# deu439/ARFlow

Measured on AMD Instinct MI355X. Metric: image-pairs/sec fwd+bwd, PWCLite 384x640 bs=8, higher is better.
Workload: dtype f32; 1 GPU; pwclite_uflow+uflow_loss, 384x640 pairs, batch 8 per GPU, fwd(both directions)+loss+bwd+allreduce+Adam; global_batch=8, parallelism=dp1, step_start=seeded weights + fresh Adam state, restored before every step, loss_finite=True

## Files before the change

arflow_amd/_lib.py:

```python
import ctypes
import os

_HERE = os.path.dirname(os.path.abspath(__file__))
LIB_PATH = os.path.join(_HERE, 'csrc', 'libarflow_hip.so')

c_fp = ctypes.c_void_p
c_i = ctypes.c_int
c_l = ctypes.c_long
c_f = ctypes.c_float
c_d = ctypes.c_double

PROTOTYPES = {
    'arflow_abi_version': [],
    'arflow_take_stale_error': [],
    'arflow_set_deterministic': [c_i],
    'arflow_get_deterministic': [],
    'arflow_flow_up_fwd': [c_fp, c_fp, c_i, c_i, c_i, c_i, c_i, c_fp],
    'arflow_flow_up_bwd': [c_fp, c_fp, c_i, c_i, c_i, c_i, c_i, c_fp],
    'arflow_out_up2_fwd': [c_fp, c_l, c_fp, c_l, c_i, c_i, c_i, c_i, c_i, c_i, c_f, c_fp],
    'arflow_out_up2_bwd': [c_fp, c_l, c_fp, c_l, c_i, c_i, c_i, c_i, c_i, c_fp],
    'arflow_out_tail_fwd': [c_fp, c_l, c_fp, c_fp, c_i, c_i, c_i, c_i, c_i, c_i, c_f, c_fp],
    'arflow_prob_up_fwd': [c_fp, c_l, c_fp, c_l, c_i, c_i, c_i, c_i, c_i, c_i, c_i, c_f, c_fp],
    'arflow_prob_up_bwd': [c_fp, c_l, c_fp, c_l, c_i, c_i, c_i, c_i, c_i, c_i, c_fp],
    'arflow_profile_marker': [c_i, c_fp],
    'arflow_sums_rows': [c_i, c_i, c_i],
    'arflow_corr_fwd': [c_fp, c_fp, c_fp, c_fp, c_i, c_i, c_i, c_i, c_i, c_f, c_fp],
    'arflow_corr_sign_planes': [c_i, c_i, c_i],
    'arflow_corr_strided_supported': [c_i, c_i, c_i],
    'arflow_corr_fwd_strided': [c_fp, c_fp, c_fp, c_l, c_fp, c_i, c_i, c_i, c_i, c_i, c_f, c_fp],
    'arflow_corr_bwd_strided': [c_fp, c_l, c_fp, c_l, c_fp, c_fp, c_fp, c_fp, c_fp, c_i, c_i, c_i, c_i, c_i, c_f, c_fp],
    'arflow_corr_bwd': [c_fp, c_fp, c_fp, c_fp, c_fp, c_fp, c_fp, c_i, c_i, c_i, c_i, c_i, c_f, c_fp],
    'arflow_corr_fwd_bf16': [c_fp, c_fp, c_fp, c_i, c_i, c_i, c_i, c_i, c_f, c_fp],
    'arflow_corr_bwd_bf16': [c_fp, c_fp, c_fp, c_fp, c_fp, c_fp, c_i, c_i, c_i, c_i, c_i, c_f, c_fp],
    'arflow_warp_fwd_bf16': [c_fp, c_fp, c_fp, c_fp, c_i, c_i, c_i, c_i, c_i, c_i, c_l, c_i, c_i, c_i, c_fp],
    'arflow_warp_bwd_bf16': [c_fp, c_fp, c_fp, c_fp, c_fp, c_i, c_i, c_i, c_i, c_i, c_i, c_l, c_i, c_i, c_i, c_fp],
    'arflow_warp_nearest_fwd': [c_fp, c_fp, c_fp, c_i, c_i, c_i, c_i, c_i, c_i, c_l, c_i, c_i, c_i, c_fp],
    'arflow_warp_nearest_bwd': [c_fp, c_fp, c_fp, c_i, c_i, c_i, c_i, c_i, c_i, c_l, c_i, c_i, c_i, c_fp],
    'arflow_warp_bicubic_fwd': [c_fp, c_fp, c_fp, c_i, c_i, c_i, c_i, c_i, c_i, c_l, c_i, c_i, c_i, c_fp],
    'arflow_warp_bicubic_bwd': [c_fp, c_fp, c_fp, c_fp, c_fp, c_i, c_i, c_i, c_i, c_i, c_i, c_l, c_i, c_i, c_i, c_fp],
    'arflow_ssim_fwd': [c_fp, c_fp, c_fp, c_i, c_i, c_i, c_i, c_i, c_fp],
    'arflow_ssim_bwd': [c_fp, c_fp, c_fp, c_fp, c_i, c_i, c_i, c_i, c_i, c_fp],
    'arflow_corr_general_out_size': [c_i, c_i, c_i, c_i, c_i, c_i, c_i, c_fp, c_fp, c_fp],
    'arflow_corr_general_fwd': [c_fp, c_fp, c_fp, c_i, c_i, c_i, c_i, c_i, c_i, c_i, c_i, c_i, c_fp],
    'arflow_corr_general_bwd': [c_fp, c_fp, c_fp, c_fp, c_fp, c_i, c_i, c_i, c_i, c_i, c_i, c_i, c_i, c_i, c_fp],
    'arflow_featnorm_fwd': [c_fp, c_fp, c_fp, c_fp, c_fp, c_fp, c_i, c_l, c_i, c_fp],
    'arflow_featnorm_bwd': [c_fp, c_fp, c_fp, c_fp, c_fp, c_fp, c_fp, c_fp, c_i, c_l, c_i, c_fp],
    'arflow_level_supported': [c_i, c_i, c_i],
    'arflow_level_bwd_ws_bytes': [c_i, c_i, c_i, c_i],
    'arflow_level_fwd': [c_fp, c_fp, c_fp, c_l, c_i, c_i, c_fp, c_fp, c_l, c_fp, c_i, c_fp, c_l, c_fp, c_l, c_fp, c_fp, c_fp, c_i, c_i, c_i, c_i, c_i, c_f, c_i, c_i, c_i, c_fp],
    'arflow_level_bwd': [c_fp, c_l, c_fp, c_fp, c_l, c_fp, c_l, c_fp, c_fp, c_fp, c_fp, c_l, c_fp, c_l, c_fp, c_fp, c_i, c_fp, c_fp, c_fp, c_i, c_i, c_fp, c_i, c_i, c_i, c_i, c_i, c_f, c_i, c_i, c_i, c_fp],
    'arflow_level_fwd_m': [c_fp, c_fp, c_fp, c_l, c_i, c_i, c_fp, c_fp, c_l, c_fp, c_i, c_fp, c_l, c_fp, c_l, c_fp, c_fp, c_fp, c_fp, c_i, c_fp, c_i, c_i, c_i, c_i, c_i, c_i, c_f, c_i, c_i, c_i, c_fp],
    'arflow_up2_bwd': [c_fp, c_fp, c_i, c_i, c_i, c_i, c_fp],
    'arflow_bias_act_mom_rows': [c_i, c_l],
    'arflow_bias_act_fwd_mom': [c_fp, c_fp, c_fp, c_fp, c_i, c_i, c_l, c_f, c_fp],
    'arflow_level_acc_rows': [c_i, c_i, c_i, c_i, c_i],
    'arflow_level_moments': [c_fp, c_fp, c_fp, c_i, c_l, c_fp],
    'arflow_level_warp_fwd': [c_fp, c_fp, c_fp, c_l, c_i, c_i, c_fp, c_fp, c_l, c_fp, c_fp, c_i, c_i, c_i, c_i, c_i, c_i, c_i, c_fp],
    'arflow_level_corr_fwd': [c_fp, c_fp, c_fp, c_i, c_i, c_fp, c_l, c_fp, c_l, c_fp, c_fp, c_i, c_i, c_i, c_i, c_i, c_f, c_fp],
    'arflow_level_corr_bwd': [c_fp, c_l, c_fp, c_fp, c_l, c_fp, c_fp, c_fp, c_fp, c_i, c_i, c_i, c_i, c_i, c_f, c_fp],
    'arflow_bias_act_fwd': [c_fp, c_fp, c_fp, c_i, c_i, c_l, c_f, c_fp],
    'arflow_bias_act_bwd': [c_fp, c_fp, c_fp, c_fp, c_i, c_i, c_l, c_f, c_fp],
    'arflow_headconv_fwd': [c_fp, c_fp, c_fp, c_fp, c_i, c_i, c_i, c_i, c_fp],
    'arflow_headconv_bwd_data': [c_fp, c_fp, c_fp, c_i, c_i, c_i, c_i, c_fp],
    'arflow_headconv_bwd_weight_ws_bytes': [c_i, c_i, c_i, c_i],
    'arflow_headconv_bwd_weight': [c_fp, c_fp, c_fp, c_fp, c_fp, c_i, c_i, c_i, c_i, c_fp],
    'arflow_splitconv_pack_bytes': [c_i, c_i],
    'arflow_splitconv_pack': [c_fp, c_fp, c_i, c_i, c_i, c_fp],
    'arflow_splitconv_fwd': [c_fp, c_fp, c_fp, c_i, c_i, c_i, c_i, c_i, c_fp],
    'arflow_splitconv_fwd_ex': [c_fp, c_l, c_fp, c_fp, c_l, c_fp, c_i, c_f, c_i, c_i, c_i, c_i, c_i, c_fp],
    'arflow_splitconv_wgrad_ws_bytes': [c_i, c_i, c_i, c_i, c_i],
    'arflow_splitconv_wgrad': [c_fp, c_l, c_fp, c_l, c_fp, c_fp, c_i, c_i, c_i, c_i, c_i, c_fp],
    'arflow_dense_cat_fwd': [c_fp, c_fp, c_fp, c_fp, c_i, c_i, c_i, c_l, c_f, c_fp],
    'arflow_dense_gbias_rows': [c_i, c_l],
    'arflow_dense_grad_gather': [c_fp, c_i, c_fp, c_l, c_fp, c_fp, c_i, c_i, c_l, c_f, c_fp],
    'arflow_warp_fwd': [c_fp, c_fp, c_fp, c_fp, c_i, c_i, c_i, c_i, c_i, c_i, c_l, c_i, c_i, c_i, c_fp],
    'arflow_warp_bwd': [c_fp, c_fp, c_fp, c_fp, c_fp, c_i, c_i, c_i, c_i, c_i, c_i, c_l, c_i, c_i, c_i, c_fp],
    'arflow_splat_map': [c_fp, c_fp, c_i, c_i, c_i, c_l, c_i, c_fp],
    'arflow_coord_mask': [c_fp, c_fp, c_i, c_i, c_i, c_l, c_i, c_fp],
    'arflow_occ_bidir': [c_fp, c_fp, c_fp, c_i, c_i, c_i, c_l, c_l, c_f, c_f, c_fp],
    'arflow_census_fwd': [c_fp, c_fp, c_fp, c_fp, c_fp, c_fp, c_i, c_i, c_i, c_i, c_fp],
    'arflow_census_bwd': [c_fp, c_fp, c_fp, c_fp, c_fp, c_i, c_i, c_i, c_i, c_fp],
    'arflow_census_warp_supported': [c_i, c_i],
    'arflow_census_warp_fwd': [c_fp, c_fp, c_fp, c_l, c_fp, c_fp, c_fp, c_fp, c_i, c_i, c_i, c_i, c_fp],
    'arflow_census_warp_bwd': [c_fp, c_fp, c_fp, c_l, c_fp, c_fp, c_fp, c_i, c_i, c_i, c_i, c_fp],
    'arflow_census_warp_pair_fwd': [c_fp, c_fp, c_l, c_fp, c_fp, c_fp, c_fp, c_i, c_i, c_i, c_i, c_fp],
    'arflow_census_warp_pair_bwd': [c_fp, c_fp, c_l, c_fp, c_fp, c_fp, c_i, c_i, c_i, c_i, c_fp],
    'arflow_uflow_pair_bwd': [c_fp, c_fp, c_l, c_fp, c_fp, c_fp, c_i, c_i, c_i, c_i, c_fp, c_l, c_fp, c_fp, c_fp, c_i, c_i, c_f, c_f, c_i, c_i, c_i, c_fp],
    'arflow_down4_gray_z': [c_fp, c_fp, c_fp, c_fp, c_i, c_i, c_i, c_fp],
    'arflow_splat_smooth_fwd': [c_fp, c_fp, c_fp, c_fp, c_i, c_i, c_i, c_l, c_f, c_f, c_i, c_i, c_i, c_i, c_fp],
    'arflow_down4_gray': [c_fp, c_fp, c_fp, c_i, c_i, c_i, c_fp],
    'arflow_photo_fwd': [c_fp, c_fp, c_fp, c_fp, c_fp, c_i, c_i, c_i, c_i, c_fp],
    'arflow_photo_bwd': [c_fp, c_fp, c_fp, c_fp, c_fp, c_fp, c_i, c_i, c_i, c_i, c_fp],
    'arflow_photo_warp_rows': [c_i, c_i, c_i],
    'arflow_photo_warp_fwd': [c_fp, c_l, c_l, c_fp, c_l, c_l, c_fp, c_l, c_l, c_fp, c_l, c_l, c_i, c_i, c_i, c_i, c_fp, c_fp, c_i, c_i, c_i, c_i, c_i, c_i, c_fp],
    'arflow_photo_warp_bwd': [c_fp, c_l, c_l, c_fp, c_l, c_l, c_fp, c_l, c_l, c_fp, c_l, c_l, c_i, c_i, c_i, c_i, c_fp, c_fp, c_l, c_l, c_i, c_i, c_i, c_i, c_i, c_i, c_fp],
    'arflow_area_pyramid_ws_bytes': [c_i, c_i, c_i, c_fp, c_i],
    'arflow_area_pyramid': [c_fp, c_fp, c_i, c_i, c_i, c_fp, c_i, c_fp],
    'arflow_smooth_fwd': [c_fp, c_fp, c_fp, c_i, c_i, c_i, c_i, c_l, c_f, c_f, c_i, c_i, c_i, c_fp],
    'arflow_smooth_bwd': [c_fp, c_fp, c_fp, c_fp, c_i, c_i, c_i, c_i, c_l, c_f, c_f, c_i, c_i, c_i, c_fp],
    'arflow_down4': [c_fp, c_fp, c_i, c_i, c_i, c_fp],
    'arflow_up4_clamp_mul': [c_fp, c_fp, c_fp, c_i, c_i, c_i, c_fp],
    'arflow_flow_eval_rows': [c_i, c_i],
    'arflow_flow_eval': [c_fp, c_fp, c_fp, c_fp, c_fp, c_i, c_i, c_i, c_i, c_i, c_i, c_fp],
    'arflow_triag_solve': [c_fp, c_fp, c_fp, c_fp, c_fp, c_fp, c_i, c_i, c_i, c_i, c_fp],
    'arflow_triag_solve_bwd': [c_fp, c_fp, c_fp, c_fp, c_fp, c_fp, c_fp, c_fp, c_fp, c_fp, c_fp, c_i, c_i, c_i, c_i, c_fp],
    'arflow_triag_inverse_diagonal': [c_fp, c_fp, c_fp, c_fp, c_i, c_i, c_i, c_fp],
    'arflow_band_mv_fwd': [c_fp, c_l, c_fp, c_l, c_fp, c_l, c_fp, c_l, c_fp, c_l, c_i, c_i, c_i, c_i, c_i, c_i, c_fp],
    'arflow_band_mv_bwd': [c_fp, c_l, c_fp, c_l, c_fp, c_l, c_fp, c_l, c_fp, c_l, c_fp, c_l, c_fp, c_l, c_fp, c_l, c_i, c_i, c_i, c_i, c_i, c_i, c_fp],
    'arflow_lowrank_sample_fwd': [c_fp, c_l, c_fp, c_l, c_fp, c_fp, c_l, c_i, c_i, c_i, c_i, c_i, c_fp],
    'arflow_lowrank_work_size': [c_i, c_i, c_i, c_i],
    'arflow_lowrank_logdet_fwd': [c_fp, c_l, c_fp, c_fp, c_fp, c_i, c_i, c_i, c_i, c_fp],
    'arflow_lowrank_bwd': [c_fp, c_l, c_fp, c_fp, c_l, c_fp, c_fp, c_fp, c_l, c_fp, c_l, c_i, c_i, c_i, c_i, c_i, c_fp],
    'arflow_mixture_work_size': [c_i, c_i, c_i, c_i, c_i],
    'arflow_mixture_sample_fwd': [c_fp, c_l, c_fp, c_l, c_fp, c_l, c_fp, c_fp, c_l, c_fp, c_i, c_i, c_i, c_i, c_i, c_fp],
    'arflow_mixture_logpdf_fwd': [c_fp, c_fp, c_fp, c_fp, c_fp, c_i, c_i, c_i, c_i, c_i, c_fp],
    'arflow_mixture_bwd': [c_fp, c_l, c_fp, c_l, c_fp, c_l, c_fp, c_fp, c_fp, c_fp, c_l, c_fp, c_l, c_fp, c_l, c_i, c_i, c_i, c_i, c_i, c_fp],
    'arflow_mixture_entropy_map': [c_fp, c_l, c_fp, c_l, c_fp, c_fp, c_fp, c_l, c_fp, c_i, c_i, c_i, c_i, c_i, c_fp],
    'arflow_gauss_pyr_work_size': [c_fp, c_fp, c_i, c_i],
    'arflow_gauss_pyr_sample_fwd': [c_fp, c_fp, c_fp, c_fp, c_fp, c_fp, c_fp, c_fp, c_i, c_i, c_fp, c_fp, c_fp],
    'arflow_gauss_pyr_sample_bwd': [c_fp, c_fp, c_fp, c_fp, c_fp, c_fp, c_fp, c_fp, c_fp, c_fp, c_fp, c_i, c_i, c_fp],
    'arflow_mse_work_size': [c_i, c_i, c_i],
    'arflow_mse_fwd': [c_fp, c_l, c_i, c_fp, c_l, c_i, c_i, c_fp, c_l, c_i, c_i, c_i, c_i, c_i, c_i, c_fp, c_fp, c_fp],
    'arflow_mse_bwd': [c_fp, c_l, c_i, c_fp, c_l, c_i, c_i, c_fp, c_l, c_fp, c_fp, c_l, c_fp, c_l, c_i, c_i, c_i, c_i, c_i, c_i, c_fp],
    'arflow_resize_flow': [c_fp, c_l, c_i, c_i, c_fp, c_l, c_i, c_i, c_i, c_i, c_fp],
# ... 56 lines not shown
```

arflow_amd/csrc/split_tiles.hpp:

```cpp
#pragma once
#include <array>

namespace splitbf16 {
inline int tiles32(int n) { return (n + 31) / 32; }
constexpr int MAX_KT = 2;

struct TilePart { int kt, count, first; };
inline std::array<TilePart, 2> split_tiles(int n, int max_t) {
  const int chunks = (n + max_t - 1) / max_t, base = n / chunks, extra = n % chunks;
  return {{{base + 1, extra, 0}, {base, chunks - extra, extra * (base + 1)}}};
}
}
```

arflow_amd/csrc/splitconv.hip:

```cpp
#include <climits>
#include <cstdint>

#include "splitbf16.hpp"

namespace {
using namespace splitbf16;

constexpr int NT = 256;
constexpr int CB = 32;
constexpr int PLANE_BYTES = CB * 2;
constexpr int PIX_BYTES = 3 * PLANE_BYTES + 16;
constexpr int FRAG = 64 * 8;

template <int PW>
struct Geo {
  static constexpr int PR = 32 / PW;
  static constexpr int TH = 8 * PR;
  static constexpr int HW = PW + 2;
  static constexpr int HH = TH + 2;
  static constexpr int NPIX = HH * HW;
  static constexpr int LDS_BYTES = NPIX * PIX_BYTES;
};

__global__ __launch_bounds__(NT) void splitconv_pack_kernel(const float* __restrict__ w, bf16x8* __restrict__ packed, int wK, int wC,
// ... 237 lines not shown
int launch(const Ends& ends, const bf16x8* packed, int N, int C, int K, int H, int W, int kt_first, int chunks, hipStream_t st) {
  using G = Geo<PW>;
  if (const int rc = allow_dynamic_lds<&splitconv_kernel<KT, PW>>(G::LDS_BYTES)) return rc;
  const int tx = (W + PW - 1) / PW, ty = (H + G::TH - 1) / G::TH;
  const dim3 grid((unsigned)((long)N * tx * ty), (unsigned)chunks);
  hipLaunchKernelGGL((splitconv_kernel<KT, PW>), grid, dim3(NT), G::LDS_BYTES, st, ends.x, ends.x_bs, packed, ends.y, ends.y_bs, ends.bias,
                     ends.act, ends.slope, C, K, H, W, tiles32(K), 2 * tiles32(C), kt_first, tx, ty);
  return af_launch_status();
}

template <int PW>
int launch_kt(int KT, const Ends& e, const bf16x8* packed, int N, int C, int K, int H, int W, int kt_first, int chunks,
              hipStream_t st) {
  return KT == 1 ? launch<1, PW>(e, packed, N, C, K, H, W, kt_first, chunks, st)
                 : launch<2, PW>(e, packed, N, C, K, H, W, kt_first, chunks, st);
}
}

extern "C" long arflow_splitconv_pack_bytes(int K, int C) {
  if (!pack_shape_ok(K, C)) return ARFLOW_ESHAPE;
  return (long)3 * 9 * tiles32(K) * 2 * tiles32(C) * FRAG * 2;
}

extern "C" int arflow_splitconv_pack(const float* w, void* packed, int K, int C, int transpose_flip, arflow_stream_t stream) {
  af_clear_stale_error();
  AF_REQUIRE_PTR(w);
  AF_REQUIRE_PTR(packed);
  AF_REQUIRE(pack_shape_ok(K, C), ARFLOW_ESHAPE);
  AF_REQUIRE(transpose_flip == 0 || transpose_flip == 1, ARFLOW_EPARAM);
  AF_REQUIRE(((uintptr_t)packed & 15) == 0, ARFLOW_EPARAM);
  const int Kout = transpose_flip ? C : K, Cin = transpose_flip ? K : C;
  const int nkt = tiles32(Kout), ncs = 2 * tiles32(Cin);
  const int nfrag = 9 * nkt * ncs * 64;
  hipLaunchKernelGGL(splitconv_pack_kernel, dim3((unsigned)af_cdiv(nfrag, NT)), dim3(NT), 0, (hipStream_t)stream, w,
                     (bf16x8*)packed, K, C, Kout, Cin, nkt, ncs, transpose_flip);
  return af_launch_status();
}

extern "C" int arflow_splitconv_fwd_ex(const float* x, long x_bstride, const void* packed, float* y, long y_bstride,
                                       const float* bias, int act, float negative_slope, int N, int C, int K, int H, int W,
                                       arflow_stream_t stream) {
  af_clear_stale_error();
  AF_REQUIRE_PTR(x);
  AF_REQUIRE_PTR(packed);
  AF_REQUIRE_PTR(y);
  AF_REQUIRE(N > 0 && C > 0 && K > 0 && H > 0 && W > 0, ARFLOW_ESHAPE);
  AF_REQUIRE((long)N * C * H * W <= INT_MAX && (long)N * K * H * W <= INT_MAX && pack_shape_ok(K, C), ARFLOW_ESHAPE);
  AF_REQUIRE(x_bstride >= (long)C * H * W && y_bstride >= (long)K * H * W, ARFLOW_ESHAPE);
  AF_REQUIRE(x_bstride <= INT_MAX / N && y_bstride <= INT_MAX / N, ARFLOW_ESHAPE);
  AF_REQUIRE(act == 0 || act == 1, ARFLOW_EPARAM);
  AF_REQUIRE(act == 1 || bias == nullptr, ARFLOW_EPARAM);
  AF_REQUIRE(((uintptr_t)packed & 15) == 0, ARFLOW_EPARAM);
  const Ends ends{x, x_bstride, y, y_bstride, bias, act, negative_slope};
  const auto waste = [&](int pw) {
    const int th = 8 * (32 / pw);
    return (long)((W + pw - 1) / pw * pw) * ((H + th - 1) / th * th);
  };
  int PW = 32;
  if (waste(16) < waste(PW)) PW = 16;
  if (waste(8) < waste(PW)) PW = 8;
  const bf16x8* pk = (const bf16x8*)packed;
  hipStream_t st = (hipStream_t)stream;
  for (const TilePart& p : split_tiles(tiles32(K), MAX_KT)) {
    if (p.count == 0) continue;
    int rc;
    if (PW == 32) rc = launch_kt<32>(p.kt, ends, pk, N, C, K, H, W, p.first, p.count, st);
    else if (PW == 16) rc = launch_kt<16>(p.kt, ends, pk, N, C, K, H, W, p.first, p.count, st);
    else rc = launch_kt<8>(p.kt, ends, pk, N, C, K, H, W, p.first, p.count, st);
    if (rc != ARFLOW_OK) return rc;
  }
  return ARFLOW_OK;
}

extern "C" int arflow_splitconv_fwd(const float* x, const void* packed, float* y, int N, int C, int K, int H, int W,
                                    arflow_stream_t stream) {
  return arflow_splitconv_fwd_ex(x, (long)C * H * W, packed, y, (long)K * H * W, nullptr, 0, 0.f, N, C, K, H, W, stream);
}
```

arflow_amd/functional.py:

```python
import contextlib

import torch

from . import _lib
from . import ddp as _ddp

PAD = {'zeros': 0, 'border': 1}
NORM_ARFLOW, NORM_UFLOW = 0, 1


def _need_gpu(*tensors):
    for t in tensors:
        if t is None:
            continue
        if not t.is_cuda:
            raise _lib.ArflowHipError('arflow_amd ops run on the GPU only (got a %s tensor); there is no CPU '
                                      'fallback -- the CPU oracle lives in oracle/ and is test-only' % t.device)
        if t.dtype != torch.float32:
            raise _lib.ArflowHipError('arflow_amd ops are fp32 only (got %s)' % t.dtype)


def _p(t):
    return None if t is None else t.data_ptr()

# ... 874 lines not shown
            ctx.save_for_backward(*xs, *ws, w_head)
        ctx.slope, ctx.inplace = slope, inplace
        ctx.set_materialize_grads(False)
        return x6, flow

    @staticmethod
    @torch.autograd.function.once_differentiable
    def backward(ctx, gx6, gflow):
        if ctx.inplace:
            x6, ws, w_head = ctx.saved_tensors[0], ctx.saved_tensors[1:6], ctx.saved_tensors[6]
            tail = [int(w.shape[0]) for w in ws]
            xs = [x6[:, sum(tail[m:]):] for m in range(5)] + [x6]
        else:
            xs, ws, w_head = ctx.saved_tensors[:6], ctx.saved_tensors[6:11], ctx.saved_tensors[11]
        need = ctx.needs_input_grad
        grads = [None] * 14
        if gx6 is None and gflow is None:
            return tuple(grads)
        x6 = xs[5]
        B, C6, H, W = x6.shape
        ocs = [int(w.shape[0]) for w in ws]
        lowest = 0 if need[0] else next((m for m in range(1, 6) if need[2 * m] or need[2 * m + 1]), 6)
        dx_head = None
        if gflow is not None:
            gflow = gflow.contiguous()
            if lowest < 6:
                dx_head = _headconv_dgrad(gflow, w_head, x6)
            grads[12], grads[13] = _headconv_wgrad(x6, gflow, w_head, need[12], need[13])
        if lowest == 6:
            return tuple(grads)
        top = [t for t in (gx6, dx_head) if t is not None]
        dxs = []
        for m in range(5, max(lowest, 1) - 1, -1):
            srcs = [(t, sum(ocs[m:5]), None) for t in top] + [(dx, sum(ocs[m:k - 1]), None) for dx, k in dxs]
            gy, gb = dense_grad_gather(srcs, ocs[m - 1], act=xs[m], slope=ctx.slope, want_bias=need[2 * m + 1])
            want_dx, want_dw = m > lowest, bool(need[2 * m])
            xm = xs[m - 1]
            dx_native = want_dx and splitconv_takes(B, ocs[m - 1], xm.shape[1], H, W)
            dw_native = want_dw and (_inplace_wgrad_takes if ctx.inplace else splitconv_wgrad_takes)(B, xm.shape[1], ocs[m - 1], H, W)
            dx, dw = _conv3x3_grads(xm, ws[m - 1], gy, want_dx, want_dw, dx_native, dw_native)
            grads[2 * m], grads[2 * m + 1] = dw, gb
            if want_dx:
                dxs.append((dx, m))
        if need[0]:
            srcs = [(t, sum(ocs), None) for t in top] + [(dx, sum(ocs[:k - 1]), None) for dx, k in dxs]
            grads[0] = dense_grad_gather(srcs, int(xs[0].shape[1]))[0]
        return tuple(grads)


def dense_estimator(x, slope, params):
    return DenseEstimatorFunction.apply(x, slope, *params)


@_samples_mode
class BiasLeakyReLUMomentsFunction(torch.autograd.Function):

    @staticmethod
    def forward(ctx, x, bias, slope):
        _need_gpu(x)
        if not x.is_contiguous():
            raise ValueError('bias_leaky_relu expects a contiguous [B,C,...] tensor')
        B, C = x.shape[0], x.shape[1]
        hw = x[0, 0].numel()
        if bias is not None:
            _need_gpu(bias)
            bias = bias.contiguous()
        rows = _lib.load().arflow_bias_act_mom_rows(C, hw)
        mom = torch.empty(B, rows, 2, device=x.device, dtype=torch.float64)
        with torch.cuda.device_of(x):
            _call('arflow_bias_act_fwd_mom', _p(x), _p(bias), _p(x), _p(mom), B, C, hw, float(slope), _stream(), key=(B, C, hw))
        ctx.mark_dirty(x)
        ctx.mark_non_differentiable(mom)
        ctx.save_for_backward(x)
        ctx.slope, ctx.has_bias = float(slope), bias is not None
        return x, mom

    @staticmethod
    def backward(ctx, gout, gmom_unused):
        y, = ctx.saved_tensors
        B, C = y.shape[0], y.shape[1]
        hw = y[0, 0].numel()
        gout = gout.contiguous()
        gin = torch.empty_like(gout)
        gb = torch.empty(C, device=y.device, dtype=torch.float32) if (ctx.has_bias and ctx.needs_input_grad[1]) else None
        with torch.cuda.device_of(y):
            _call('arflow_bias_act_bwd', _p(gout), _p(y), _p(gin), _p(gb), B, C, hw, ctx.slope, _stream(), key=(B, C, hw))
        return gin, gb, None


def bias_leaky_relu_moments(x, bias, slope=0.1):
    return BiasLeakyReLUMomentsFunction.apply(x, bias, slope)


@_samples_mode
class WarpFunction(torch.autograd.Function):

    @staticmethod
    def forward(ctx, src, flow, pad, align_corners, norm, want_valid=False):
        _need_gpu(src, flow)
        src = src.contiguous()
        flow, fbs = _flow_view(flow)
        B, C, Hs, Ws = src.shape
        _, _, H, W = flow.shape
        if flow.shape[0] != B:
            raise ValueError('batch mismatch between source and flow')
        out = torch.empty(B, C, H, W, device=src.device, dtype=torch.float32)
# ... 1041 lines not shown
```

arflow_amd/models/blocks.py:

```python
import torch
import torch.nn as nn
import torch.nn.functional as F

from .. import functional as AF

bias_act = AF.bias_leaky_relu


class ConvAct(nn.Sequential):

    want_moments = False
    last_moments = None

    def split_route(self, x):
        if not self._split_kind(x):
            return False, False
        c = self[0]
        N, C, H, W = x.shape
        return AF.splitconv_takes(N, C, c.out_channels, H, W), AF.splitconv_takes(N, c.out_channels, C, H, W)

    def split_wgrad_route(self, x):
        if not self._split_kind(x):
            return False
        N, C, H, W = x.shape
# ... 78 lines not shown

    def __init__(self, ch_in, ch_out=2):
        super().__init__()
        self.conv1 = conv(ch_in, 128)
        self.conv2 = conv(ch_in + 128, 128)
        self.conv3 = conv(ch_in + 256, 96)
        self.conv4 = conv(ch_in + 352, 64)
        self.conv5 = conv(ch_in + 416, 32)
        self.feat_dim = ch_in + 448
        self.conv_last = conv(ch_in + 448, ch_out, isReLU=False)

    def native(self, x):
        return AF.dense_block_enabled() and self.conv_last.native(x) and self.conv1[0].weight.dtype == torch.float32

    def forward(self, x):
        layers = (self.conv1, self.conv2, self.conv3, self.conv4, self.conv5)
        if self.native(x):
            params = [p for layer in layers + (self.conv_last,) for p in (layer[0].weight, layer[0].bias)]
            return AF.dense_estimator(x, self.conv1[1].negative_slope, params)
        for layer in layers:
            x = torch.cat([layer(x), x], dim=1)
        return x, self.conv_last(x)


class FlowEstimatorReduce(nn.Module):

    def __init__(self, ch_in, ch_out=2):
        super().__init__()
        self.conv1 = conv(ch_in, 128)
        self.conv2 = conv(128, 128)
        self.conv3 = conv(128 + 128, 96)
        self.conv4 = conv(128 + 96, 64)
        self.conv5 = conv(96 + 64, 32)
        self.feat_dim = 32
        self.predict_flow = conv(64 + 32, ch_out, isReLU=False)

    def forward(self, x):
        x1 = self.conv1(x)
        x2 = self.conv2(x1)
        x3 = self.conv3(torch.cat([x1, x2], dim=1))
        x4 = self.conv4(torch.cat([x2, x3], dim=1))
        x5 = self.conv5(torch.cat([x3, x4], dim=1))
        return x5, self.predict_flow(torch.cat([x4, x5], dim=1))


class ContextNetwork(nn.Module):

    def __init__(self, ch_in, ch_out=2):
        super().__init__()
        self.convs = nn.Sequential(
            conv(ch_in, 128, 3, 1, 1), conv(128, 128, 3, 1, 2), conv(128, 128, 3, 1, 4), conv(128, 96, 3, 1, 8),
            conv(96, 64, 3, 1, 16), conv(64, 32, 3, 1, 1), conv(32, ch_out, isReLU=False))

    def forward(self, x):
        return self.convs(x)


def init_conv_weights(module, scheme):
    for layer in module.modules():
        if isinstance(layer, (nn.Conv2d, nn.ConvTranspose2d)):
            if scheme == 'kaiming':
                nn.init.kaiming_normal_(layer.weight)
            else:
                nn.init.xavier_uniform_(layer.weight)
            if layer.bias is not None:
                nn.init.constant_(layer.bias, 0)


def level_drops(training, rate, n, n_passes, batch_per_pass, device):
    if not (training and rate > 0):
        return None
    vals = [[float(torch.rand(1) > rate) for _ in range(n)] for _ in range(n_passes)]
    t = torch.tensor(vals, dtype=torch.float32)
    t = t.repeat_interleave(batch_per_pass, dim=0).t().contiguous()
    return t.to(device, non_blocking=True).view(n, -1, 1, 1, 1)


def pair_pass(pyr_all, moms, B, with_bk, run):
    have_m = moms is not None and all(t is not None for t in moms)
    if with_bk:
        swapped = [torch.cat([p[B:], p[:B]], 0) for p in pyr_all]
        m = (list(moms), [torch.roll(t, B, 0) for t in moms]) if have_m else None
        flows = run(list(pyr_all), swapped, 2, m)
        return {'flows_fw': [f[:B] for f in flows], 'flows_bw': [f[B:] for f in flows]}
    m = ([t[:B] for t in moms], [t[B:] for t in moms]) if have_m else None
    return {'flows_fw': run([p[:B] for p in pyr_all], [p[B:] for p in pyr_all], 1, m)}
```

include/arflow_hip.h:

```cpp
#ifndef ARFLOW_HIP_H
#define ARFLOW_HIP_H

#ifdef __cplusplus
extern "C" {
#endif

typedef void* arflow_stream_t;

#define ARFLOW_OK 0
#define ARFLOW_ENULL (-1001)
#define ARFLOW_ESHAPE (-1002)
#define ARFLOW_EPARAM (-1003)
#define ARFLOW_ENONDET (-1004)
#define ARFLOW_ELAUNCH_BASE (-2000)

#define ARFLOW_PAD_ZEROS 0
#define ARFLOW_PAD_BORDER 1

#define ARFLOW_NORM_ARFLOW 0
#define ARFLOW_NORM_UFLOW 1
#define ARFLOW_NORM_UFLOW_ABS 2
#define ARFLOW_COORDS_ABS 2

#define ARFLOW_SUM_COLS 4
// ... 56 lines not shown
int arflow_level_fwd_m(const float* x1, const float* x2, const float* flow, long flow_bstride, int flow_is_coarse,
                       int up_align_corners, float* flow_up, float* flow_up2, long flow_up2_bstride, float* x2w, int norm_mode,
                       float* out, long out_bstride, float* x1n, long x1n_bstride, unsigned* sign_bits, float* stats,
                       double* acc, const double* x1_rows, int x1_nrows, const double* x2_rows, int x2_nrows, int B, int C, int H,
                       int W, int max_disp, float negative_slope, int pad_mode, int align_corners, int coord_norm,
                       arflow_stream_t stream);
int arflow_level_bwd(const float* gout, long gout_bstride, const unsigned* sign_bits, const float* x1n, long x1n_bstride,
                     const float* gx1n_direct, long gx1n_direct_bstride, const float* x1, const float* x2, const float* x2w,
                     const float* flow_full, long flow_bstride, const float* gflow_a, long gflow_a_bstride,
                     const float* gflow_b, const float* stats, int norm_mode, float* gx1, float* gx2, float* gflow,
                     int flow_is_coarse, int up_align_corners, void* workspace, int B, int C, int H, int W, int max_disp,
                     float negative_slope, int pad_mode, int align_corners, int coord_norm, arflow_stream_t stream);
int arflow_level_acc_rows(int B, int C, int H, int W, int has_flow);
int arflow_up2_bwd(const float* gfine, float* gcoarse, int B, int H, int W, int up_align_corners, arflow_stream_t stream);
int arflow_level_moments(const float* x1, const float* x2, double* acc, int B, long n, arflow_stream_t stream);
int arflow_level_warp_fwd(const float* x1, const float* x2, const float* flow, long flow_bstride, int flow_is_coarse,
                          int up_align_corners, float* flow_up, float* flow_up2, long flow_up2_bstride, float* x2w,
                          double* acc, int B, int C, int H, int W, int pad_mode, int align_corners, int norm_mode,
                          arflow_stream_t stream);
int arflow_level_corr_fwd(const float* x1, const float* x2w, const double* acc, int acc_rows, int norm_mode, float* out,
                          long out_bstride, float* x1n, long x1n_bstride, unsigned* sign_bits, float* stats, int B, int C,
                          int H, int W, int max_disp, float negative_slope, arflow_stream_t stream);
int arflow_level_corr_bwd(const float* gout, long gout_bstride, const unsigned* sign_bits, const float* x1n,
                          long x1n_bstride, const float* x2w, const float* stats, float* gx1n, float* gx2n, int B, int C,
                          int H, int W, int max_disp, float negative_slope, arflow_stream_t stream);

int arflow_bias_act_fwd(const float* x, const float* bias, float* y, int B, int C, long HW,
                        float negative_slope, arflow_stream_t stream);
int arflow_bias_act_mom_rows(int C, long HW);
int arflow_bias_act_fwd_mom(const float* x, const float* bias, float* y, double* mom, int B, int C, long HW,
                            float negative_slope, arflow_stream_t stream);
int arflow_bias_act_bwd(const float* gout, const float* y, float* gin, float* gbias, int B, int C, long HW,
                        float negative_slope, arflow_stream_t stream);

int arflow_headconv_fwd(const float* x, const float* w, const float* bias, float* y, int B, int C, int H, int W,
                        arflow_stream_t stream);
int arflow_headconv_bwd_data(const float* dy, const float* w, float* dx, int B, int C, int H, int W,
                             arflow_stream_t stream);
long arflow_headconv_bwd_weight_ws_bytes(int B, int C, int H, int W);
int arflow_headconv_bwd_weight(const float* x, const float* dy, float* dw, float* dbias, void* ws, int B, int C, int H,
                               int W, arflow_stream_t stream);

long arflow_splitconv_pack_bytes(int K, int C);
int arflow_splitconv_pack(const float* w, void* packed, int K, int C, int transpose_flip, arflow_stream_t stream);
int arflow_splitconv_fwd(const float* x, const void* packed, float* y, int N, int C, int K, int H, int W,
                         arflow_stream_t stream);

int arflow_splitconv_fwd_ex(const float* x, long x_bstride, const void* packed, float* y, long y_bstride, const float* bias,
                            int act, float negative_slope, int N, int C, int K, int H, int W, arflow_stream_t stream);

long arflow_splitconv_wgrad_ws_bytes(int N, int C, int K, int H, int W);
int arflow_splitconv_wgrad(const float* x, long x_bstride, const float* dy, long dy_bstride, float* dw, void* ws, int N, int C,
                           int K, int H, int W, arflow_stream_t stream);

#define ARFLOW_DENSE_MAX_SRC 8
typedef struct {
  const float* ptr;
  long bstride;
  const float* scale;
} arflow_dense_src;
int arflow_dense_cat_fwd(const float* y, const float* bias, const float* x, float* out, int B, int oc, int C, long HW,
                         float negative_slope, arflow_stream_t stream);
int arflow_dense_gbias_rows(int B, long HW);
int arflow_dense_grad_gather(const arflow_dense_src* srcs, int n_src, const float* act, long act_bs, float* gy,
                             float* gbias_rows, int B, int oc, long HW, float negative_slope, arflow_stream_t stream);

int arflow_warp_fwd(const float* src, const float* flow, float* out, float* valid, int B, int C,
                    int Hs, int Ws, int H, int W, long flow_bstride, int pad_mode, int align_corners,
                    int norm_mode, arflow_stream_t stream);

int arflow_warp_bwd(const float* gout, const float* src, const float* flow, float* gsrc, float* gflow,
                    int B, int C, int Hs, int Ws, int H, int W, long flow_bstride, int pad_mode,
                    int align_corners, int norm_mode, arflow_stream_t stream);

int arflow_splat_map(const float* flow, float* out, int B, int H, int W, long flow_bstride,
                     int variant, arflow_stream_t stream);

int arflow_coord_mask(const float* flow, float* out, int B, int H, int W, long flow_bstride, int mode,
                      arflow_stream_t stream);

int arflow_occ_bidir(const float* flow12, const float* flow21, float* out, int B, int H, int W,
                     long bstride12, long bstride21, float scale, float bias, arflow_stream_t stream);

int arflow_census_fwd(const float* im_a, const float* im_b, const float* mask, float* ham, float* dham,
                      float* sums, int B, int H, int W, int radius, arflow_stream_t stream);

int arflow_census_bwd(const float* im_a, const float* im_b, const float* gham, const float* scale,
                      float* g_im_b, int B, int H, int W, int radius, arflow_stream_t stream);

int arflow_census_warp_supported(int H, int W);
int arflow_census_warp_fwd(const float* gray_a, const float* gray_b, const float* flow, long flow_bstride,
                           const float* occ_small, float* mask_out, float* dham, float* sums, int B, int H, int W,
                           int radius, arflow_stream_t stream);
int arflow_census_warp_bwd(const float* gray_a, const float* gray_b, const float* flow, long flow_bstride,
                           const float* dham, const float* scale, float* gflow, int B, int H, int W, int radius,
                           arflow_stream_t stream);
int arflow_census_warp_pair_fwd(const float* gray, const float* flow, long flow_bstride, const float* occ_small,
                                float* mask_out, float* dham, float* sums, int B2, int H, int W, int radius,
                                arflow_stream_t stream);
int arflow_census_warp_pair_bwd(const float* gray, const float* flow, long flow_bstride, const float* dham,
                                const float* scale2, float* gflow, int B2, int H, int W, int radius, arflow_stream_t stream);
int arflow_uflow_pair_bwd(const float* gray, const float* flow, long flow_bstride, const float* dham, const float* scale2,
                          float* gflow, int B2, int H, int W, int radius, const float* flow2, long flow2_bstride,
                          const float* img2, const float* coef2, float* gflow2, int h2, int w2, float flow_scale, float alpha,
                          int order, int wmode, int penalty, arflow_stream_t stream);
int arflow_down4_gray(const float* im, float* small, float* gray, int B, int H, int W, arflow_stream_t stream);
// ... 190 lines not shown
```

Before: 190.6 image-pairs/s.

## Run dilated context-network convs as dense convs in a phase-decomposed layout

Adds phase kernels that rearrange activations into a space-to-batch (phase-decomposed) layout, so each dilated 3x3 conv in the context network becomes an ordinary dense 3x3 conv. These can then run on the existing bf16-split splitconv kernel instead of the framework's dilated convolution path. A custom autograd function chains the four dilated layers. It fuses the phase reshuffle with the leaky-ReLU backward and the bias-gradient reduction, and falls back to MIOpen weight-gradient on the plain layout for some layers. The trade is extra layout-conversion passes, padding in the virtual layout, and more saved tensors, in exchange for faster dense conv kernels.

```diff
diff --git a/arflow_amd/_lib.py b/arflow_amd/_lib.py
--- a/arflow_amd/_lib.py
+++ b/arflow_amd/_lib.py
@@ -70,6 +70,10 @@
     'arflow_splitconv_fwd_ex': [c_fp, c_l, c_fp, c_fp, c_l, c_fp, c_i, c_f, c_i, c_i, c_i, c_i, c_i, c_fp],
     'arflow_splitconv_wgrad_ws_bytes': [c_i, c_i, c_i, c_i, c_i],
     'arflow_splitconv_wgrad': [c_fp, c_l, c_fp, c_l, c_fp, c_fp, c_i, c_i, c_i, c_i, c_i, c_fp],
+    'arflow_phase_layout': [c_i, c_i, c_i, c_i, c_fp],
+    'arflow_phase_rows': [c_i, c_i, c_i, c_i, c_i],
+    'arflow_phase_move': [c_fp, c_fp, c_fp, c_i, c_i, c_i, c_i, c_i, c_i, c_i, c_fp],
+    'arflow_phase_act_bwd': [c_fp, c_fp, c_fp, c_fp, c_fp, c_i, c_i, c_i, c_i, c_i, c_i, c_i, c_f, c_fp],
     'arflow_dense_cat_fwd': [c_fp, c_fp, c_fp, c_fp, c_i, c_i, c_i, c_l, c_f, c_fp],
     'arflow_dense_gbias_rows': [c_i, c_l],
     'arflow_dense_grad_gather': [c_fp, c_i, c_fp, c_l, c_fp, c_fp, c_i, c_i, c_l, c_f, c_fp],
diff --git a/arflow_amd/csrc/phase.hip b/arflow_amd/csrc/phase.hip
--- /dev/null
+++ b/arflow_amd/csrc/phase.hip
@@ -0,0 +1,174 @@
+#include <climits>
+
+#include "common.hpp"
+#include "phase_plan.hpp"
+
+namespace {
+using phase_plan::Plan;
+
+constexpr int NT = 256, NW = NT / 64;
+constexpr int RW = 8;
+constexpr int RB = RW * NW;
+constexpr int MAX_LDS = 160 * 1024 - 128;
+
+struct Ent {
+  int off;
+  int w;
+};
+struct Seg {
+  long base;
+  bool exists;
+};
+__device__ __forceinline__ Seg segments(const Plan& p, int C, int n, int c, int h) {
+  const phase_plan::Row r = phase_plan::row_to_virtual(p, h);
+  const long plane = (long)p.Hv * p.Wv;
+  Seg s;
+  s.exists = r.hv < p.Hv;
+  s.base = ((long)phase_plan::sample_to_virtual(p, n, r.g, 0) * C + c) * plane + (long)r.hv * p.Wv;
+  return s;
+}
+PHASE_HD inline int row_elements(const Plan& p) { return (p.d / p.Qg) * p.Wv; }
+PHASE_HD inline int named_rows(const Plan& p) { return (p.Pg == 1 ? p.Hs : p.Hs + 1) * p.d; }
+
+PHASE_HD inline int lds_column(int w) { return w + (w >> 5); }
+PHASE_HD inline int lds_pitch(int W) { return lds_column(W - 1) + 1; }
+
+__device__ __forceinline__ void column_map(const Plan& p, int C, Ent* __restrict__ tab) {
+  const int n = row_elements(p), step = C * p.Hv * p.Wv;
+  for (int t = threadIdx.x; t < n; t += NT) {
+    const int g = t / p.Wv, wv = t - g * p.Wv;
+    const int w = phase_plan::col_to_real(p, g, wv);
+    tab[t] = {g * step + wv, w < 0 ? -1 : lds_column(w)};
+  }
+}
+
+template <bool ACT>
+__global__ __launch_bounds__(NT) void phase_kernel(const float* __restrict__ src, const float* __restrict__ act, float* __restrict__ dst,
+                                                   float* __restrict__ dst2, double* __restrict__ rows, Plan ps, Plan pd, Plan pd2,
+                                                   int C, float slope) {
+  extern __shared__ __align__(8) float lds[];
+  __shared__ double red[NW];
+  const int lane = threadIdx.x & 63, wave = threadIdx.x >> 6;
+  const int c = blockIdx.y, n = blockIdx.z;
+  const int h0 = blockIdx.x * RB + wave * RW;
+  const int H = ps.H, W = lds_pitch(ps.W);
+  float* const mine = lds + (size_t)wave * RW * W;
+  const int nsrc = row_elements(ps), nd = row_elements(pd);
+  Ent* const tsrc = reinterpret_cast<Ent*>(lds + (size_t)RB * W);
+  Ent* const tdst = tsrc + nsrc;
+  Ent* const tdst2 = tdst + nd;
+  column_map(ps, C, tsrc);
+  column_map(pd, C, tdst);
+  if (dst2) column_map(pd2, C, tdst2);
+  __syncthreads();
+
+  double s[1] = {0.0};
+  if (h0 < H) {
+    long base[RW];
+#pragma unroll
+    for (int r = 0; r < RW; ++r) base[r] = segments(ps, C, n, c, min(h0 + r, H - 1)).base;
+    for (int t = lane; t < nsrc; t += 64) {
+      const Ent e = tsrc[t];
+      if (e.w < 0) continue;
+      float v[RW], a[RW];
+#pragma unroll
+      for (int r = 0; r < RW; ++r) {
+        v[r] = src[base[r] + e.off];
+        a[r] = ACT ? act[base[r] + e.off] : 1.f;
+      }
+#pragma unroll
+      for (int r = 0; r < RW; ++r) {
+        if (ACT) {
+          v[r] = a[r] > 0.f ? v[r] : v[r] * slope;
+          if (h0 + r < H) s[0] += (double)v[r];
+        }
+        mine[r * W + e.w] = v[r];
+      }
+    }
+  }
+  __syncthreads();
+
+  const auto put = [&](float* __restrict__ out, const Plan& p, const Ent* __restrict__ tab, int ne) {
+    const int hend = named_rows(p);
+    if (h0 >= hend) return;
+    Seg o[RW];
+#pragma unroll
+    for (int r = 0; r < RW; ++r) o[r] = segments(p, C, n, c, min(h0 + r, hend - 1));
+    for (int t = lane; t < ne; t += 64) {
+      const Ent e = tab[t];
+#pragma unroll
+      for (int r = 0; r < RW; ++r) {
+        if (h0 + r >= hend || !o[r].exists) continue;
+        out[o[r].base + e.off] = e.w >= 0 && h0 + r < H ? mine[r * W + e.w] : 0.f;
+      }
+    }
+  };
+  put(dst, pd, tdst, nd);
+  if (dst2) put(dst2, pd2, tdst2, row_elements(pd2));
+
+  if (ACT && rows) {
+    af_block_sum_f64<1, NT>(s, red);
+    if (threadIdx.x == 0) rows[((long)n * gridDim.x + blockIdx.x) * C + c] = s[0];
+  }
+}
+
+inline int walked_rows(const Plan& pd, const Plan* pd2) {
+  int h = named_rows(pd);
+  if (pd2 && named_rows(*pd2) > h) h = named_rows(*pd2);
+  return h;
+}
+inline bool layout_ok(int N, int C, int H, int W, int d) {
+  if (!(C > 0 && C <= 65535 && N <= 65535 && phase_plan::shape_ok(N, H, W, d))) return false;
+  return phase_plan::elements(phase_plan::make_plan(N, H, W, d), C) <= INT_MAX;
+}
+
+template <bool ACT>
+int launch(const float* src, const float* act, float* dst, float* dst2, double* rows, int N, int C, int H, int W, int d_src, int d_dst,
+           int d_dst2, float slope, hipStream_t st) {
+  AF_REQUIRE(layout_ok(N, C, H, W, d_src) && layout_ok(N, C, H, W, d_dst) && (!dst2 || layout_ok(N, C, H, W, d_dst2)), ARFLOW_ESHAPE);
+  const Plan ps = phase_plan::make_plan(N, H, W, d_src), pd = phase_plan::make_plan(N, H, W, d_dst);
+  const Plan pd2 = dst2 ? phase_plan::make_plan(N, H, W, d_dst2) : pd;
+  const long bytes = sizeof(float) * (long)RB * lds_pitch(W) + sizeof(Ent) * ((long)row_elements(ps) + row_elements(pd) + (dst2 ? row_elements(pd2) : 0));
+  AF_REQUIRE(bytes <= MAX_LDS, ARFLOW_ESHAPE);
+  if (bytes > 64 * 1024) {
+    const hipError_t e = hipFuncSetAttribute(reinterpret_cast<const void*>(&phase_kernel<ACT>), hipFuncAttributeMaxDynamicSharedMemorySize, MAX_LDS);
+    if (e != hipSuccess) return af_hip_status(e);
+  }
+  const dim3 grid((unsigned)af_cdiv(walked_rows(pd, dst2 ? &pd2 : nullptr), RB), (unsigned)C, (unsigned)N);
+  hipLaunchKernelGGL(phase_kernel<ACT>, grid, dim3(NT), (size_t)bytes, st, src, act, dst, dst2, rows, ps, pd, pd2, C, slope);
+  return af_launch_status();
+}
+}
+
+extern "C" int arflow_phase_layout(int N, int H, int W, int d, int* nv_hv_wv_pg_qg) {
+  AF_REQUIRE_PTR(nv_hv_wv_pg_qg);
+  AF_REQUIRE(phase_plan::shape_ok(N, H, W, d), ARFLOW_ESHAPE);
+  const Plan p = phase_plan::make_plan(N, H, W, d);
+  nv_hv_wv_pg_qg[0] = p.Nv, nv_hv_wv_pg_qg[1] = p.Hv, nv_hv_wv_pg_qg[2] = p.Wv, nv_hv_wv_pg_qg[3] = p.Pg, nv_hv_wv_pg_qg[4] = p.Qg;
+  return ARFLOW_OK;
+}
+
+extern "C" int arflow_phase_rows(int N, int H, int W, int d_dst, int d_dst2) {
+  AF_REQUIRE(phase_plan::shape_ok(N, H, W, d_dst) && (d_dst2 == 0 || phase_plan::shape_ok(N, H, W, d_dst2)), ARFLOW_ESHAPE);
+  const Plan pd = phase_plan::make_plan(N, H, W, d_dst), pd2 = phase_plan::make_plan(N, H, W, d_dst2 ? d_dst2 : d_dst);
+  return N * af_cdiv(walked_rows(pd, &pd2), RB);
+}
+
+extern "C" int arflow_phase_move(const float* src, float* dst, float* dst2, int N, int C, int H, int W, int d_src, int d_dst,
+                                 int d_dst2, arflow_stream_t stream) {
+  af_clear_stale_error();
+  AF_REQUIRE_PTR(src);
+  AF_REQUIRE_PTR(dst);
+  AF_REQUIRE((dst2 == nullptr) == (d_dst2 == 0), ARFLOW_EPARAM);
+  return launch<false>(src, nullptr, dst, dst2, nullptr, N, C, H, W, d_src, d_dst, d_dst2, 0.f, (hipStream_t)stream);
+}
+
+extern "C" int arflow_phase_act_bwd(const float* gout, const float* y, float* gin, float* gin2, double* rows, int N, int C, int H,
+                                    int W, int d_a, int d_b, int d_b2, float negative_slope, arflow_stream_t stream) {
+  af_clear_stale_error();
+  AF_REQUIRE_PTR(gout);
+  AF_REQUIRE_PTR(y);
+  AF_REQUIRE_PTR(gin);
+  AF_REQUIRE((gin2 == nullptr) == (d_b2 == 0), ARFLOW_EPARAM);
+  return launch<true>(gout, y, gin, gin2, rows, N, C, H, W, d_a, d_b, d_b2, negative_slope, (hipStream_t)stream);
+}
diff --git a/arflow_amd/csrc/phase_plan.hpp b/arflow_amd/csrc/phase_plan.hpp
--- /dev/null
+++ b/arflow_amd/csrc/phase_plan.hpp
@@ -0,0 +1,89 @@
+#pragma once
+#include <climits>
+
+#include "split_tiles.hpp"
+
+#if defined(__HIPCC__)
+#define PHASE_HD __host__ __device__
+#else
+#define PHASE_HD
+#endif
+
+namespace phase_plan {
+struct Plan {
+  int N, H, W, d;
+  int Pg, Qg;
+  int Hs, Ws;
+  int Hv, Wv, Nv;
+};
+
+inline bool shape_ok(int N, int H, int W, int d) { return N > 0 && H > 0 && W > 0 && d > 0 && d <= H && d <= W && (long)N * d * d <= INT_MAX; }
+
+inline Plan with_groups(int N, int H, int W, int d, int Pg, int Qg) {
+  Plan p;
+  p.N = N, p.H = H, p.W = W, p.d = d, p.Pg = Pg, p.Qg = Qg;
+  p.Hs = (H + d - 1) / d, p.Ws = (W + d - 1) / d;
+  p.Hv = Pg * (p.Hs + 1) - 1, p.Wv = Qg * (p.Ws + 1) - 1;
+  p.Nv = N * (d / Pg) * (d / Qg);
+  return p;
+}
+inline long tiled_pixels(const Plan& p) {
+  return (long)(p.d / p.Pg) * (p.d / p.Qg) * splitbf16::tile_pixels(p.Hv, p.Wv, splitbf16::pixel_tile_width(p.Hv, p.Wv));
+}
+inline Plan make_plan(int N, int H, int W, int d) {
+  Plan best = with_groups(N, H, W, d, 1, 1);
+  for (int Pg = 1; Pg <= d; ++Pg) {
+    if (d % Pg) continue;
+    for (int Qg = 1; Qg <= d; ++Qg) {
+      if (d % Qg) continue;
+      const Plan c = with_groups(N, H, W, d, Pg, Qg);
+      const long cc = tiled_pixels(c), cb = tiled_pixels(best);
+      if (cc < cb || (cc == cb && Pg * Qg < best.Pg * best.Qg)) best = c;
+    }
+  }
+  return best;
+}
+inline long elements(const Plan& p, int C) { return (long)p.Nv * C * p.Hv * p.Wv; }
+
+struct Row {
+  int g, hv;
+};
+PHASE_HD inline Row row_to_virtual(const Plan& p, int h) {
+  const int ph = h % p.d;
+  return {ph / p.Pg, (ph % p.Pg) * (p.Hs + 1) + h / p.d};
+}
+struct Col {
+  int g, wv;
+};
+PHASE_HD inline Col col_to_virtual(const Plan& p, int w) {
+  const int ph = w % p.d;
+  return {ph / p.Qg, (ph % p.Qg) * (p.Ws + 1) + w / p.d};
+}
+PHASE_HD inline int row_to_real(const Plan& p, int g, int hv) {
+  const int a = hv / (p.Hs + 1), i = hv % (p.Hs + 1);
+  const int h = i * p.d + g * p.Pg + a;
+  return i < p.Hs && h < p.H ? h : -1;
+}
+PHASE_HD inline int col_to_real(const Plan& p, int g, int wv) {
+  const int b = wv / (p.Ws + 1), j = wv % (p.Ws + 1);
+  const int w = j * p.d + g * p.Qg + b;
+  return j < p.Ws && w < p.W ? w : -1;
+}
+PHASE_HD inline int sample_to_virtual(const Plan& p, int n, int gp, int gq) { return (n * (p.d / p.Pg) + gp) * (p.d / p.Qg) + gq; }
+
+struct Pos {
+  int n, h, w;
+};
+PHASE_HD inline Pos to_virtual(const Plan& p, int n, int h, int w) {
+  const Row r = row_to_virtual(p, h);
+  const Col c = col_to_virtual(p, w);
+  return {sample_to_virtual(p, n, r.g, c.g), r.hv, c.wv};
+}
+PHASE_HD inline bool to_real(const Plan& p, int nv, int hv, int wv, Pos& o) {
+  const int nq = p.d / p.Qg, np = p.d / p.Pg;
+  const int h = row_to_real(p, (nv / nq) % np, hv), w = col_to_real(p, nv % nq, wv);
+  if (h < 0 || w < 0) return false;
+  o = {nv / (nq * np), h, w};
+  return true;
+}
+}
diff --git a/arflow_amd/csrc/split_tiles.hpp b/arflow_amd/csrc/split_tiles.hpp
--- a/arflow_amd/csrc/split_tiles.hpp
+++ b/arflow_amd/csrc/split_tiles.hpp
@@ -10,4 +10,15 @@
   const int chunks = (n + max_t - 1) / max_t, base = n / chunks, extra = n % chunks;
   return {{{base + 1, extra, 0}, {base, chunks - extra, extra * (base + 1)}}};
 }
+
+inline long tile_pixels(int H, int W, int pw) {
+  const int th = 8 * (32 / pw);
+  return (long)((W + pw - 1) / pw * pw) * ((H + th - 1) / th * th);
 }
+inline int pixel_tile_width(int H, int W) {
+  int pw = 32;
+  if (tile_pixels(H, W, 16) < tile_pixels(H, W, pw)) pw = 16;
+  if (tile_pixels(H, W, 8) < tile_pixels(H, W, pw)) pw = 8;
+  return pw;
+}
+}
diff --git a/arflow_amd/csrc/splitconv.hip b/arflow_amd/csrc/splitconv.hip
--- a/arflow_amd/csrc/splitconv.hip
+++ b/arflow_amd/csrc/splitconv.hip
@@ -313,13 +313,7 @@
   AF_REQUIRE(act == 1 || bias == nullptr, ARFLOW_EPARAM);
   AF_REQUIRE(((uintptr_t)packed & 15) == 0, ARFLOW_EPARAM);
   const Ends ends{x, x_bstride, y, y_bstride, bias, act, negative_slope};
-  const auto waste = [&](int pw) {
-    const int th = 8 * (32 / pw);
-    return (long)((W + pw - 1) / pw * pw) * ((H + th - 1) / th * th);
-  };
-  int PW = 32;
-  if (waste(16) < waste(PW)) PW = 16;
-  if (waste(8) < waste(PW)) PW = 8;
+  const int PW = pixel_tile_width(H, W);
   const bf16x8* pk = (const bf16x8*)packed;
   hipStream_t st = (hipStream_t)stream;
   for (const TilePart& p : split_tiles(tiles32(K), MAX_KT)) {
diff --git a/arflow_amd/functional.py b/arflow_amd/functional.py
--- a/arflow_amd/functional.py
+++ b/arflow_amd/functional.py
@@ -950,6 +950,146 @@
     return DenseEstimatorFunction.apply(x, slope, *params)
 
 
+_DILATED_CHAIN = __import__('os').environ.get('ARFLOW_DILATED_CHAIN', '1') != '0'
+DILATED_CHAIN_LAYERS = ((128, 128, 2), (128, 128, 4), (128, 96, 8), (96, 64, 16))
+_DILATED_WGRAD_NATIVE = (True, False, False, False)
+
+
+def dilated_chain_enabled():
+    return _DILATED_CHAIN
+
+
+def _dilated_wgrad_native():
+    env = __import__('os').environ.get('ARFLOW_DILATED_WGRAD')
+    if env and len(env) == 4 and set(env) <= {'0', '1'}:
+        return tuple(c == '1' for c in env)
+    return _DILATED_WGRAD_NATIVE
+
+
+def phase_layout(N, H, W, d):
+    import ctypes
+    out = (ctypes.c_int * 5)()
+    _lib.check(_lib.load().arflow_phase_layout(int(N), int(H), int(W), int(d), ctypes.cast(out, ctypes.c_void_p)), 'arflow_phase_layout')
+    return tuple(out)
+
+
+def _phase_empty(N, C, H, W, d, device):
+    if d == 1:
+        return torch.empty(N, C, H, W, device=device, dtype=torch.float32)
+    Nv, Hv, Wv, _, _ = phase_layout(N, H, W, d)
+    return torch.empty(Nv, C, Hv, Wv, device=device, dtype=torch.float32)
+
+
+def _phase_check(t, N, H, W, d, what):
+    _need_gpu(t)
+    Nv, Hv, Wv, _, _ = phase_layout(N, H, W, d)
+    if t.dim() != 4 or (t.shape[0], t.shape[2], t.shape[3]) != (Nv, Hv, Wv) or not t.is_contiguous():
+        raise ValueError('%s must be a contiguous [%d,C,%d,%d] tensor: layout %d of [%d,C,%d,%d]' % (what, Nv, Hv, Wv, d, N, H, W))
+
+
+def phase_move(src, real, d_src, d_dst, d_dst2=0, out=None, out2=None):
+    N, H, W = (int(v) for v in real)
+    _phase_check(src, N, H, W, d_src, 'phase_move: src')
+    C = int(src.shape[1])
+    dst = _phase_empty(N, C, H, W, d_dst, src.device) if out is None else out
+    dst2 = (_phase_empty(N, C, H, W, d_dst2, src.device) if out2 is None else out2) if d_dst2 else None
+    for t, d in ((out, d_dst), (out2 if d_dst2 else None, d_dst2)):
+        if t is not None:
+            _phase_check(t, N, H, W, d, 'phase_move: out')
+            if t.shape[1] != C:
+                raise ValueError('phase_move: out has %d channels, src %d' % (t.shape[1], C))
+    with torch.cuda.device_of(src):
+        _call('arflow_phase_move', _p(src), _p(dst), _p(dst2), N, C, H, W, int(d_src), int(d_dst), int(d_dst2), _stream())
+    return dst, dst2
+
+
+def phase_act_bwd(gout, y, real, d_a, d_b, d_b2=0, slope=0.1, want_bias=True):
+    N, H, W = (int(v) for v in real)
+    _phase_check(gout, N, H, W, d_a, 'phase_act_bwd: gout')
+    _phase_check(y, N, H, W, d_a, 'phase_act_bwd: y')
+    if y.shape != gout.shape:
+        raise ValueError('phase_act_bwd: gout and y differ in shape')
+    C = int(gout.shape[1])
+    gin = _phase_empty(N, C, H, W, d_b, gout.device)
+    gin2 = _phase_empty(N, C, H, W, d_b2, gout.device) if d_b2 else None
+    rows = None
+    if want_bias:
+        n = _lib.load().arflow_phase_rows(N, H, W, int(d_b), int(d_b2))
+        if n <= 0:
+            _lib.check(n, 'arflow_phase_rows')
+        rows = torch.empty(n, C, device=gout.device, dtype=torch.float64)
+    with torch.cuda.device_of(gout):
+        _call('arflow_phase_act_bwd', _p(gout), _p(y), _p(gin), _p(gin2), _p(rows), N, C, H, W, int(d_a), int(d_b), int(d_b2),
+              float(slope), _stream())
+    return gin, gin2, (None if rows is None else rows.sum(0).float())
+
+
+def _dilated_wgrad_miopen(x, gy, w, d):
+    args = [1, 1], [d, d], [d, d], False, [0, 0], 1
+    return torch.ops.aten.convolution_backward(gy, x, w, None, *args, [False, True, False])[1]
+
+
+class DilatedChainFunction(torch.autograd.Function):
+
+    @staticmethod
+    def forward(ctx, x, slope, *params):
+        if len(params) != 8:
+            raise ValueError('dilated_chain expects (w, b) of four layers')
+        _need_gpu(x, *params)
+        ws, bs = params[0::2], params[1::2]
+        shapes = tuple((int(w.shape[1]), int(w.shape[0]), d) for w, (_, _, d) in zip(ws, DILATED_CHAIN_LAYERS))
+        if shapes != DILATED_CHAIN_LAYERS or x.dim() != 4 or x.shape[1] != shapes[0][0]:
+            raise ValueError('dilated_chain: the layers are %s' % (DILATED_CHAIN_LAYERS,))
+        slope = float(slope)
+        ds = [d for _, _, d in DILATED_CHAIN_LAYERS]
+        native = _dilated_wgrad_native()
+        x = x.contiguous()
+        N, _, H, W = x.shape
+        real = (N, H, W)
+        a, _ = phase_move(x, real, 1, ds[0])
+        ins, plain = [], [x]
+        for k in range(4):
+            ins.append(a)
+            y = splitconv(a, ws[k], bias=bs[k], slope=slope)
+            if k == 3:
+                a, _ = phase_move(y, real, ds[k], 1)
+            else:
+                a, a_plain = phase_move(y, real, ds[k], ds[k + 1], 0 if native[k + 1] else 1)
+                plain.append(a_plain)
+        ctx.save_for_backward(a, *ins, *plain, *ws)
+        ctx.slope, ctx.real, ctx.native = slope, real, native
+        return a
+
+    @staticmethod
+    @torch.autograd.function.once_differentiable
+    def backward(ctx, gout):
+        saved = ctx.saved_tensors
+        out, ins, plain, ws = saved[0], saved[1:5], saved[5:9], saved[9:13]
+        need = ctx.needs_input_grad
+        ds = [d for _, _, d in DILATED_CHAIN_LAYERS]
+        grads = [None] * 10
+        g, lay, yk = gout.contiguous(), 1, out
+        for k in range(3, -1, -1):
+            want_dw, want_db = need[2 + 2 * k], need[3 + 2 * k]
+            native = ctx.native[k] or not want_dw
+            gin, gin_plain, grads[3 + 2 * k] = phase_act_bwd(g, yk, ctx.real, lay, ds[k], 0 if native else 1, ctx.slope, want_db)
+            if want_dw:
+                grads[2 + 2 * k] = splitconv_wgrad(ins[k], gin) if native else _dilated_wgrad_miopen(plain[k], gin_plain, ws[k], ds[k])
+            if k > 0 or need[0]:
+                g, lay, yk = splitconv(gin, ws[k], transpose_flip=True), ds[k], ins[k]
+        if need[0]:
+            grads[0] = phase_move(g, ctx.real, ds[0], 1)[0]
+        return tuple(grads)
+
+
+def dilated_chain(x, slope, params):
+    return DilatedChainFunction.apply(x, slope, *params)
+
+
+def dilated_chain_takes(N, H, W):
+    return _SPLITCONV and _DILATED_CHAIN and _size_floor(int(N), int(H), int(W), 96, 160)
+
+
 @_samples_mode
 class BiasLeakyReLUMomentsFunction(torch.autograd.Function):
 
diff --git a/arflow_amd/models/blocks.py b/arflow_amd/models/blocks.py
--- a/arflow_amd/models/blocks.py
+++ b/arflow_amd/models/blocks.py
@@ -154,8 +154,24 @@
             conv(ch_in, 128, 3, 1, 1), conv(128, 128, 3, 1, 2), conv(128, 128, 3, 1, 4), conv(128, 96, 3, 1, 8),
             conv(96, 64, 3, 1, 16), conv(64, 32, 3, 1, 1), conv(32, ch_out, isReLU=False))
 
-    def forward(self, x):
-        return self.convs(x)
+    def native(self, x):
+        if not (bias_act is AF.bias_leaky_relu and x.is_cuda and x.dtype == torch.float32 and x.dim() == 4):
+            return False
+        convs = [layer[0] for layer in self.convs[1:5]]
+        kind = all(c.weight.dtype == torch.float32 and c.kernel_size == (3, 3) and c.stride == (1, 1) and c.padding == c.dilation and
+                   c.dilation[0] == c.dilation[1] and c.groups == 1 and c.padding_mode == 'zeros' and c.bias is not None for c in convs)
+        shapes = tuple((c.in_channels, c.out_channels, c.dilation[0]) for c in convs)
+        slopes = {layer[1].negative_slope for layer in self.convs[1:5]}
+        return (kind and shapes == AF.DILATED_CHAIN_LAYERS and len(slopes) == 1 and
+                AF.dilated_chain_takes(x.shape[0], x.shape[2], x.shape[3]))
+
+    def forward(self, x):
+        if not self.native(x):
+            return self.convs(x)
+        x = self.convs[0](x)
+        params = [p for layer in self.convs[1:5] for p in (layer[0].weight, layer[0].bias)]
+        x = AF.dilated_chain(x, self.convs[1][1].negative_slope, params)
+        return self.convs[6](self.convs[5](x))
 
 
 def init_conv_weights(module, scheme):
diff --git a/include/arflow_hip.h b/include/arflow_hip.h
--- a/include/arflow_hip.h
+++ b/include/arflow_hip.h
@@ -132,6 +132,13 @@
 long arflow_splitconv_wgrad_ws_bytes(int N, int C, int K, int H, int W);
 int arflow_splitconv_wgrad(const float* x, long x_bstride, const float* dy, long dy_bstride, float* dw, void* ws, int N, int C,
                            int K, int H, int W, arflow_stream_t stream);
+
+int arflow_phase_layout(int N, int H, int W, int d, int* nv_hv_wv_pg_qg);
+int arflow_phase_rows(int N, int H, int W, int d_dst, int d_dst2);
+int arflow_phase_move(const float* src, float* dst, float* dst2, int N, int C, int H, int W, int d_src, int d_dst, int d_dst2,
+                      arflow_stream_t stream);
+int arflow_phase_act_bwd(const float* gout, const float* y, float* gin, float* gin2, double* rows, int N, int C, int H, int W,
+                         int d_a, int d_b, int d_b2, float negative_slope, arflow_stream_t stream);
 
 #define ARFLOW_DENSE_MAX_SRC 8
 typedef struct {
```

New measurement: 195.8 image-pairs/s (median of 6 runs). 2.8% higher.
